# Vigilans/GomokuAI

Hardware: AMD Instinct MI355X
Metric: board-evals/s (higher is better)
Workload: dtype int32; 1 GPU; batched AC-automaton position eval (K1), 65536 random-opening boards per GPU, 15x15, inputs resident in HBM; boards_per_gpu=65536, parallelism=boards sharded by rank, no collective, launch=hipGraph replay of the K steps

## Files before the change

### gomokuai_amd/csrc/eval_kernel.hip

```cpp
#include <algorithm>
#include <cstdlib>
#include <vector>

#include "capi_common.h"
#include "host_staging.h"

namespace {

constexpr int kBoardsPerBlock = 16;
constexpr int kGroupBoards = 16;
constexpr int kThreads = 64 * kBoardsPerBlock;
constexpr int kCells = 225;
constexpr int kQueueCap = 448;
constexpr int kMaxBlocksPerCu = 1;
constexpr int kBurstEvery = 12;
static_assert(kBurstEvery >= 1 && kBurstEvery <= kGroupBoards, "every burst of a run needs a board of the run to go with");
[[maybe_unused]] constexpr int kTimelineSlots = 8;

constexpr int kScoreWords = 4 * kCells;
constexpr int kCntWords = 3 * kCells + 1;
constexpr int kZeroWords = kScoreWords + kCntWords;
constexpr int kLineWords = 96;
constexpr int kColBase = 20, kDiagBase = 36, kAntiBase = 65;
#ifndef GMK_K1_TOTALS_COPIES
#define GMK_K1_TOTALS_COPIES 8
#endif
constexpr int kTotalsCopies = GMK_K1_TOTALS_COPIES;
constexpr int kMiscWords = 48;
constexpr int kBoardWords = kZeroWords + kLineWords + kQueueCap + kMiscWords;
static_assert(kZeroWords % 4 == 0 && kBoardWords % 4 == 0, "16-byte alignment of the per-board blocks");
constexpr int kStaticTableWords = 128 + kLineWords + 512 + 1560 + 4;

constexpr int kLaneRecordVecs = 2;
constexpr int kScanSteps = 19;

__device__ __forceinline__ int dir_stride(int dir) { return (0x0E100F01u >> (8 * dir)) & 0xFFu; }

__device__ __forceinline__ uint64_t line_symbols(uint32_t line_word, int len) {
    return 2ull | (static_cast<uint64_t>(line_word) << 2) | (0xAull << (2 * len + 2));
}

__device__ __forceinline__ const __attribute__((address_space(3))) uint32_t* lds_word(uint32_t byte_address) {
    return reinterpret_cast<const __attribute__((address_space(3))) uint32_t*>(static_cast<uintptr_t>(byte_address));
}

__device__ __forceinline__ __attribute__((address_space(3))) uint32_t* lds_word_rw(uint32_t byte_address) {
    return reinterpret_cast<__attribute__((address_space(3))) uint32_t*>(static_cast<uintptr_t>(byte_address));
}

__device__ __forceinline__ uint32_t dfa_address(uint32_t table_word, uint32_t four) {
    uint32_t addr;
    asm("v_bfi_b32 %0, %1, %2, %3" : "=v"(addr) : "s"(0x3FF3u), "v"(table_word), "v"(four));
    return addr;
}

typedef unsigned short v2u16 __attribute__((ext_vector_type(2)));
__device__ __forceinline__ uint32_t pk_dec_u16(uint32_t word) {
    const v2u16 ones = {1, 1};
    return __builtin_bit_cast(uint32_t, static_cast<v2u16>(__builtin_bit_cast(v2u16, word) - ones));
}

__device__ __forceinline__ void store_saddr(uint32_t byte_offset, int32_t value, unsigned long long base) {
    asm volatile("global_store_dword %0, %1, %2" : : "v"(byte_offset), "v"(value), "s"(base) : "memory");
}

template <int kImm, bool kNt>
__device__ __forceinline__ void store_saddr_imm(uint32_t byte_offset, int32_t value, unsigned long long base) {
    static_assert(kImm >= 0 && kImm < 4096, "the immediate offset of a global store has 13 bits, signed");
    if (kNt) asm volatile("global_store_dword %0, %1, %2 offset:%3 nt" : : "v"(byte_offset), "v"(value), "s"(base), "n"(kImm) : "memory");
    else asm volatile("global_store_dword %0, %1, %2 offset:%3" : : "v"(byte_offset), "v"(value), "s"(base), "n"(kImm) : "memory");
}

__device__ __forceinline__ void wave_phase_fence() {
    __builtin_amdgcn_fence(__ATOMIC_RELEASE, "wavefront");
    __builtin_amdgcn_wave_barrier();
    __builtin_amdgcn_fence(__ATOMIC_ACQUIRE, "wavefront");
}

__device__ __forceinline__ void deposit_match(uint32_t w0, uint32_t w1, int cell_at, int dir, int back_step,
                                              uint32_t* s_scores, uint32_t* s_cnt, uint32_t* s_misc, uint32_t* totals ) {
    const int type = w0 & 15, fav = (w0 >> 4) & 1;
    if (type == 8) { atomicOr(&s_misc[1], fav ? 1u : 2u); return; }
    atomicAdd(&totals[type], fav ? 0x10000u : 1u);
    const int endcell = cell_at + static_cast<int>((w0 >> 27) & 1u) * back_step;
    const uint32_t score = dir >= 2 ? (w1 >> 16) : (w1 & 0xFFFFu);
    unsigned long long* pair = reinterpret_cast<unsigned long long*>(s_scores) + fav;
    const uint32_t lo_opp = fav ? score : 0u, hi_opp = fav ? 0u : score;
    const uint32_t tslot = 5u - static_cast<uint32_t>(type);
    const bool feeds = tslot < 3u;
    uint32_t* cnt = s_cnt + (feeds ? tslot : 0u) * kCells;
    const uint32_t one = 1u << (4 * (fav * 4 + dir));
    const int n_dep = (w0 >> 8) & 7;
#pragma unroll
    for (int d = 0; d < 4; ++d) {
        if (d >= n_dep) break;
        const uint32_t f = (w0 >> (11 + 4 * d)) & 15u;
        const int c = endcell + static_cast<int>(f & 7u) * back_step;
        const bool both = (f & 8u) != 0u;
        atomicAdd(&pair[2 * c], (static_cast<unsigned long long>(both ? score : hi_opp) << 32) | (both ? score : lo_opp));
        if (both && feeds) atomicAdd(&cnt[c], one);
    }
}

__device__ __forceinline__ int counter_match(uint32_t w0, int k, int want) {
    const int type = w0 & 15, len = (w0 >> 5) & 7;
    const int back = k - static_cast<int>((w0 >> 27) & 1u) - 6;
    if (!w0 || type != want || back < 0 || back >= len) return -1;
    const int n_dep = (w0 >> 8) & 7;
    bool on_q = false;
#pragma unroll
    for (int d = 0; d < 4; ++d) {
        const uint32_t f = (w0 >> (11 + 4 * d)) & 15u;
        on_q |= d < n_dep && f == (8u | static_cast<uint32_t>(back));
    }
    return on_q ? back : -1;
}

__device__ __forceinline__ void add_counter_cells(uint32_t w0, int back, int q, int stride, uint32_t* opp) {
    const int n_dep = (w0 >> 8) & 7, endcell = q + back * stride;
#pragma unroll
    for (int d = 0; d < 4; ++d) {
        const uint32_t f = (w0 >> (11 + 4 * d)) & 15u;
// ... 71 lines not shown
    }
    if ((lane & 33) == 0) {
        const int bg = lane >> 1;
        uint32_t* slot = s_occ + 8 * ((bg >> 1) & 1) + 2 * (bg >> 2) + (bg & 1);
#pragma unroll
        for (int m = 0; m < kDensTiles; ++m) {
            const int y0 = (32 * m) / 15, y1 = (32 * m + 31) / 15;
            uint32_t occ = 0;
#pragma unroll
            for (int y = y0; y <= y1; ++y) {
                const uint32_t both = own[y / 2] | other[y / 2];
                const uint32_t r = ((y & 1) ? both >> 16 : both) & 0x7FFFu;
                const int at = 15 * y - 32 * m;
                occ |= at >= 0 ? r << at : r >> -at;
            }
            slot[16 * m] = occ;
        }
    }
    if ((lane >> 5) == 0 && (kFull || (board < n_boards && plane_stride > 0))) {
        uint32_t c224 = 0, w224 = 0;
#pragma unroll
        for (int dy = -3; dy <= 0; ++dy) {
            const int y = 14 + dy;
            const uint32_t r = (y & 1) ? own[y >> 1] >> 16 : own[y >> 1] & 0xFFFFu;
#pragma unroll
            for (int dx = -3; dx <= 0; ++dx) {
                if (block_weight(dy, dx) == 0) continue;
                const uint32_t bit = (r >> (14 + dx)) & 1u;
                c224 += bit;
                w224 += bit * static_cast<uint32_t>(block_weight(dy, dx));
            }
        }
        const uint32_t neg = 0u - (((own[7] | other[7]) >> 14) & 1u);
        int32_t* out = out_density + static_cast<size_t>(board) * 4 * plane_stride + (1 - plane) * 2 * plane_stride;
        out[224] = static_cast<int32_t>(c224 ^ neg);
        out[plane_stride + 224] = static_cast<int32_t>(w224 ^ neg);
    }
    const int n_live = __builtin_amdgcn_readfirstlane(n_boards - first_board);
    int32_t* group_out = out_density + static_cast<size_t>(first_board) * 4 * plane_stride;
    const uint4* occ_words = reinterpret_cast<const uint4*>(s_occ);
    const unsigned long long group_bits = reinterpret_cast<unsigned long long>(group_out);
    unsigned long long board_base = static_cast<unsigned long long>(static_cast<uint32_t>(__builtin_amdgcn_readfirstlane(static_cast<int>(group_bits >> 32)))) << 32
                                    | static_cast<uint32_t>(__builtin_amdgcn_readfirstlane(static_cast<int>(group_bits)));
    asm volatile("" : "+s"(board_base));
#define GMK_PASS(K, M) density_tile_pass<kFull, K, M>(own, n_live, lane, s_wtab, occ_words, group_out, board_base, s_lut, plane_stride); __builtin_amdgcn_sched_barrier(0);
    GMK_PASS(0, 0) GMK_PASS(1, 0) GMK_PASS(0, 1) GMK_PASS(1, 1) GMK_PASS(0, 2) GMK_PASS(1, 2) GMK_PASS(0, 3) GMK_PASS(1, 3)
    GMK_PASS(0, 4) GMK_PASS(1, 4) GMK_PASS(0, 5) GMK_PASS(1, 5) GMK_PASS(0, 6) GMK_PASS(1, 6)
#undef GMK_PASS
}

__global__ __launch_bounds__(kThreads)
void eval_positions_kernel(const uint16_t* __restrict__ planes, int n_boards, int groups_each, int groups_extra,
                           int32_t* __restrict__ out_scores, int32_t* __restrict__ out_density,
                           uint32_t* __restrict__ out_totals, int32_t* __restrict__ out_status,
                           const uint4* __restrict__ g_stage, int stage_vecs, int trans_words, int record_words,
                           int phase_mask_arg, unsigned long long* __restrict__ prof, unsigned long long* __restrict__ timeline) {
#ifdef GMK_PROFILE
    unsigned long long* const tl_row = timeline ? timeline + (static_cast<size_t>(blockIdx.x) * kBoardsPerBlock + (threadIdx.x >> 6)) * kTimelineSlots : nullptr;
#define GMK_TL(slot, value) do { if (tl_row && (threadIdx.x & 63) == 0) tl_row[slot] = (value); } while (0)
    GMK_TL(0, __builtin_amdgcn_s_memtime());
    unsigned long long tl_last_board = 0, tl_burst_clocks = 0;
    int tl_bursts = 0;
    const int phase_mask = phase_mask_arg;
    unsigned long long t_acc[12] = {0, 0, 0, 0, 0, 0, 0, 0, 0, 0, 0, 0}, t_prev = __builtin_amdgcn_s_memtime();
#define GMK_STAMP(k) do { if (prof) { const unsigned long long t_now_ = __builtin_amdgcn_s_memtime(); t_acc[k] += t_now_ - t_prev; t_prev = t_now_; } } while (0)
#else
    constexpr int phase_mask = 0x7F;
    (void)phase_mask_arg; (void)prof; (void)timeline;
#define GMK_TL(slot, value) do { } while (0)
#ifdef GMK_K1_MARKERS
#define GMK_STAMP(k) asm volatile("; gmk_mark " #k)
#else
#define GMK_STAMP(k) do { } while (0)
#endif
#endif
    extern __shared__ __attribute__((aligned(16))) uint32_t lds[];
    const uint4* s_rec = reinterpret_cast<const uint4*>(lds + trans_words);
    uint32_t* s_jobs = lds + trans_words + record_words;

    const int tid = threadIdx.x;
    const uint4 stage_a = g_stage[min(tid, stage_vecs - 1)], stage_b = g_stage[min(tid + kThreads, stage_vecs - 1)];
    const uint4* lane_record = g_stage + stage_vecs + kLaneRecordVecs * (tid & 63);
    const uint4 lane_lines = lane_record[0], lane_consts = lane_record[1];
    uint32_t* s_pads = s_jobs + 128;
    uint2* s_lut = reinterpret_cast<uint2*>(s_jobs + 128 + kLineWords);
    uint32_t* s_wtab_words = s_jobs + 128 + kLineWords + 512;
    const v4i* s_wtab = reinterpret_cast<const v4i*>(s_wtab_words);
    uint32_t* s_handout = s_wtab_words + kWtabWords;

    const int wave = __builtin_amdgcn_readfirstlane(threadIdx.x >> 6), lane0 = threadIdx.x & 63;
    uint32_t* s_scores = lds + trans_words + record_words + kStaticTableWords + wave * kBoardWords;
    uint32_t* s_cnt = s_scores + kScoreWords;
    uint32_t* s_lines = s_scores + kZeroWords;
    uint32_t* s_queue = s_lines + kLineWords;
    uint32_t* s_misc = s_queue + kQueueCap;
#ifndef GMK_K1_TOTALS_HOT
    uint32_t* const my_totals = s_queue + kQueueCap - 8 * kTotalsCopies + (lane0 & (kTotalsCopies - 1)) * 8;
#else
    uint32_t* const my_totals = s_misc + 4;
#endif

    GMK_STAMP(0);

    const bool planes_out = out_density != nullptr && (phase_mask & 64) && !(phase_mask & 1024);
    int lane = lane0;
    const uint32_t job_a = lane_lines.x, job_b = lane_lines.y;
    const uint32_t line_init_lo = lane_lines.z, line_init_hi = lane_lines.w;
    const uint32_t cell_row4 = lane_consts.x, cell_col = lane_consts.y, norm_a = lane_consts.z, norm_b = lane_consts.w;
    uint32_t* s_rows = s_misc + 16;
    const uint16_t* row_ptr = planes + (lane & 15);
    uint32_t next_black = 0, next_white = 0, cur_black = 0, cur_white = 0;
    auto fetch_row = [&](int b) {
        const uint16_t* p = row_ptr + static_cast<size_t>(min(b, n_boards - 1)) * 32;
        next_black = p[0];
        next_white = p[16];
    };
    auto take_row = [&](int lane_m, int b) -> uint32_t { return lane_m < 16 && b < n_boards ? cur_black | (cur_white << 16) : 0u; };

    const int wg_block = static_cast<int>(blockIdx.x);
    const int wg_g0 = groups_each * wg_block + min(wg_block, groups_extra);
    const int wg_groups = groups_each + (wg_block < groups_extra ? 1 : 0);
    const int wg_first = wg_g0 * kGroupBoards, wg_boards = min(wg_groups * kGroupBoards, n_boards - wg_first);
    auto hand_out = [&]() -> int {
        uint32_t v = 0;
        if (lane0 == 0) v = atomicAdd(s_handout, 1u);
        return __builtin_amdgcn_readfirstlane(static_cast<int>(v));
    };
    int idx = wave, boards_done = 0;
    if (idx < wg_boards) fetch_row(wg_first + idx);
    {
        uint4* s_stage = reinterpret_cast<uint4*>(lds);
        if (tid < stage_vecs) s_stage[tid] = stage_a;
        if (tid + kThreads < stage_vecs) s_stage[tid + kThreads] = stage_b;
        for (int i = tid + 2 * kThreads; i < stage_vecs; i += kThreads) s_stage[i] = g_stage[i];
    }
    asm volatile("" : "+v"(next_black), "+v"(next_white));
    GMK_TL(1, __builtin_amdgcn_s_memtime());
#pragma unroll 1
    for (;;) {
#ifdef GMK_K1_MARKERS
        GMK_STAMP(10);
#endif
        const bool live = idx < wg_boards;
        const int board = wg_first + idx;
        cur_black = next_black; cur_white = next_white;
        int idx_next = idx;
        if (live) { idx_next = boards_done == 0 ? kBoardsPerBlock + wave : hand_out(); fetch_row(wg_first + min(idx_next, wg_boards - 1)); }
        GMK_STAMP(11);

        if (live) {
            {
                uint4* z = reinterpret_cast<uint4*>(s_cnt) + lane;
    #pragma unroll
                for (int i = 0; i < kCntWords / 4; i += 64)
                    if (i + 64 <= kCntWords / 4 || lane < kCntWords / 4 - i) z[i] = make_uint4(0u, 0u, 0u, 0u);
            }
            int lane_m = lane;
            asm volatile("" : "+v"(lane_m));
            s_lines[lane] = line_init_lo;
            if (lane_m < kLineWords - 64) s_lines[64 + lane] = line_init_hi;
            if (lane_m < kMiscWords) s_misc[lane] = 0;
#ifndef GMK_K1_TOTALS_HOT
            if (lane < 8 * kTotalsCopies) s_queue[kQueueCap - 8 * kTotalsCopies + lane] = 0;
#endif
            const uint32_t my_row = take_row(lane_m, board);
            wave_phase_fence();
            {
                uint32_t cnt = static_cast<uint32_t>(__popc(my_row & 0x7FFFu)) | (static_cast<uint32_t>(__popc(my_row >> 16)) << 16);
                cnt += static_cast<uint32_t>(__builtin_amdgcn_update_dpp(0, static_cast<int>(cnt), 0x118, 0xF, 0xF, false));
                cnt += static_cast<uint32_t>(__builtin_amdgcn_update_dpp(0, static_cast<int>(cnt), 0x114, 0xF, 0xF, false));
                cnt += static_cast<uint32_t>(__builtin_amdgcn_update_dpp(0, static_cast<int>(cnt), 0x112, 0xF, 0xF, false));
                cnt += static_cast<uint32_t>(__builtin_amdgcn_update_dpp(0, static_cast<int>(cnt), 0x111, 0xF, 0xF, false));
                if (lane_m == 15) s_misc[0] = cnt;
            }
            {
                const uint32_t r = my_row;
                const v2u16 rr = __builtin_bit_cast(v2u16, r);
                const uint32_t l1 = __builtin_bit_cast(uint32_t, static_cast<v2u16>(rr << 1)), l2 = __builtin_bit_cast(uint32_t, static_cast<v2u16>(rr << 2)), l3 = __builtin_bit_cast(uint32_t, static_cast<v2u16>(rr << 3));
                const uint32_t r1 = __builtin_bit_cast(uint32_t, static_cast<v2u16>(rr >> 1)), r2 = __builtin_bit_cast(uint32_t, static_cast<v2u16>(rr >> 2)), r3 = __builtin_bit_cast(uint32_t, static_cast<v2u16>(rr >> 3));
                const int far = static_cast<int>(r | l3 | r3), near = static_cast<int>(r | l1 | l2 | r1 | r2);
                uint32_t g = l1 | l2 | l3 | r1 | r2 | r3;
                g |= static_cast<uint32_t>(__builtin_amdgcn_update_dpp(0, near, 0x111, 0xF, 0xF, true)) | static_cast<uint32_t>(__builtin_amdgcn_update_dpp(0, near, 0x101, 0xF, 0xF, true));
                g |= static_cast<uint32_t>(__builtin_amdgcn_update_dpp(0, near, 0x112, 0xF, 0xF, true)) | static_cast<uint32_t>(__builtin_amdgcn_update_dpp(0, near, 0x102, 0xF, 0xF, true));
                g |= static_cast<uint32_t>(__builtin_amdgcn_update_dpp(0, far, 0x113, 0xF, 0xF, true)) | static_cast<uint32_t>(__builtin_amdgcn_update_dpp(0, far, 0x103, 0xF, 0xF, true));
                const uint32_t empty = ~(r | (r >> 16)) & 0x7FFFu;
                if (lane < 15) s_rows[3 + lane] = r;
                const int gate = static_cast<int>(g & (empty | (empty << 16)));
    #pragma unroll
                for (int pass = 0; pass < 4; ++pass) {
                    const uint32_t gw = static_cast<uint32_t>(__builtin_amdgcn_ds_bpermute(static_cast<int>((cell_row4 >> (8 * pass)) & 0xFFu), gate)) >> ((cell_col >> (8 * pass)) & 0xFFu);
                    if (pass < 3 || lane < kCells - 192)
                        reinterpret_cast<uint4*>(s_scores)[64 * pass + lane] = make_uint4(static_cast<uint32_t>(__builtin_amdgcn_sbfe(static_cast<int>(gw), 16, 1)) & 160u, 0u, 0u,
                                                                                          static_cast<uint32_t>(__builtin_amdgcn_sbfe(static_cast<int>(gw), 0, 1)) & 160u);
                }
            }
            {
                const int y = lane >> 2, part = lane & 3;
                const uint32_t row = __shfl(my_row, min(y, 14));
                uint32_t row_sym = 0;
                uint32_t y2 = 2u * static_cast<uint32_t>(y), y4 = 4u * static_cast<uint32_t>(y);
                asm volatile("" : "+v"(y2), "+v"(y4));
                for (uint32_t m = lane < 60 ? (row | (row >> 16)) & (0xFu << (4 * part)) & 0x7FFFu : 0u; m; m &= m - 1u) {
                    const int x = __ffs(m) - 1;
                    const uint32_t code = ((row >> x) & 1u) | 2u;
                    const uint32_t at_x = code << (2 * x), at_y = code << y2;
                    row_sym |= at_x;
                    char* const col = reinterpret_cast<char*>(s_lines + x);
                    atomicXor(reinterpret_cast<uint32_t*>(col) + kColBase, at_y);
                    atomicXor(reinterpret_cast<uint32_t*>(col - y4) + (kDiagBase + 14), at_x);
                    atomicXor(reinterpret_cast<uint32_t*>(col + y4) + kAntiBase, at_y);
                }
                if (row_sym) atomicXor(&s_lines[y], row_sym);
            }
            wave_phase_fence();
            GMK_STAMP(1);
        }
#ifdef GMK_PROFILE
        if (boards_done == 0) GMK_TL(2, __builtin_amdgcn_s_memtime());
#endif
        if (boards_done == 0) __syncthreads();
#ifdef GMK_PROFILE
        if (boards_done == 0) GMK_TL(3, __builtin_amdgcn_s_memtime());
        if (live) { tl_bursts = 0; tl_burst_clocks = 0; }
#endif
        if (live) {
            int n_queued = 0;
            if (phase_mask & 2) {
                const int len_a = static_cast<int>(job_a & 31u) - 3, len_b = static_cast<int>(job_b & 31u) - 3;
                uint64_t syms = line_symbols(s_lines[(job_a >> 20) & 127u] >> norm_a, len_a);
                syms |= line_symbols(s_lines[(job_b >> 20) & 127u] >> norm_b, len_b) << (2 * len_a + 6);
                syms |= 0xAAAAAAAAAAAAAAAAull << (2 * (len_a + len_b) + 12);
                const uint32_t cur = static_cast<uint32_t>(syms) << 2;
                const uint32_t rest = static_cast<uint32_t>(syms >> 28);
                uint32_t tw = 0;
                const uint32_t q_base = static_cast<uint32_t>(s_queue - lds) * 4u;
                const uint32_t q_full = q_base + 4u * (kQueueCap - 64);
                uint32_t q_at = q_base;
                auto push = [&](uint32_t word, int step) {
                    const bool emits = word > 0x1FFFFu;
                    const unsigned long long emitters = __ballot(emits);
                    if (emitters) {
                        if (emits) {
                            const uint32_t ahead = __builtin_amdgcn_mbcnt_hi(static_cast<uint32_t>(emitters >> 32), __builtin_amdgcn_mbcnt_lo(static_cast<uint32_t>(emitters), 0u));
                            *lds_word_rw(q_at + 4u * ahead) = (word & ~0x1FFFFu) | (static_cast<uint32_t>(lane) | static_cast<uint32_t>(step) << 6);
                        }
                        q_at = min(q_at + 4u * static_cast<uint32_t>(__popcll(emitters)), q_full);
                    }
                };
#pragma unroll
                for (int step = 0; step < kScanSteps; ++step) {
                    const uint32_t four = step < 15 ? __builtin_amdgcn_ubfe(cur, 2 * step, 4) : __builtin_amdgcn_ubfe(rest, 2 * (step - 15), 4);
                    const uint32_t addr = dfa_address(tw, four);
                    const uint32_t before = tw;
                    tw = *lds_word(addr);
                    if (step > 0) push(before, step - 1);
                }
                push(tw, kScanSteps - 1);
                n_queued = static_cast<int>((q_at - q_base) >> 2);
                if (q_at >= q_full) s_misc[2] = 1;
            }
            wave_phase_fence();
            GMK_STAMP(2);

            if (phase_mask & 4) {
                uint32_t qe_next = s_queue[min(lane, kQueueCap - 1)];
                for (int m = lane; m < n_queued; m += 64) {
                    const uint32_t qe = qe_next;
                    qe_next = s_queue[min(m + 64, kQueueCap - 1)];
                    const int src_lane = qe & 63, src_step = (qe >> 6) & 31;
                    const uint4 rec_now = s_rec[qe >> 17];
                    const uint32_t ja_now = s_jobs[src_lane * 2], jb_now = s_jobs[src_lane * 2 + 1];
                    const int seg_a = ja_now & 31u;
                    const bool second = src_step >= seg_a;
                    const uint32_t job = second ? jb_now : ja_now;
                    const int pos = src_step - 1 - (second ? seg_a : 0);
                    const int dir = (job >> 5) & 3, stride = (job >> 7) & 31;
                    const int cell_at = static_cast<int>((job >> 12) & 255u) + pos * stride;
                    deposit_match(rec_now.x, rec_now.y, cell_at, dir, -stride, s_scores, s_cnt, s_misc, my_totals);
                    if (rec_now.z) deposit_match(rec_now.z, rec_now.w, cell_at, dir, -stride, s_scores, s_cnt, s_misc, my_totals);
                }
            }
            wave_phase_fence();
#ifndef GMK_K1_TOTALS_HOT
            if (lane < 8) {
                const uint32_t* t = s_queue + kQueueCap - 8 * kTotalsCopies + lane;
                uint32_t sum = 0;
#pragma unroll
                for (int c = 0; c < kTotalsCopies; ++c) sum += t[8 * c];
                s_misc[4 + lane] = sum;
            }
#endif
            GMK_STAMP(3);

            int n_cand = 0;
            if (phase_mask & 8) {
                uint32_t any_cnt[4];
    #pragma unroll
                for (int pass = 0; pass < 4; ++pass) {
                    const int qc = min(64 * pass + lane, kCells - 1);
                    any_cnt[pass] = s_cnt[qc] | s_cnt[kCells + qc] | s_cnt[2 * kCells + qc];
                }
    #pragma unroll
                for (int pass = 0; pass < 4; ++pass) {
                    const int q = 64 * pass + lane;
                    const uint32_t any = any_cnt[pass];
                    const uint32_t hot = any & (pk_dec_u16(any) | 0xEEEEEEEEu);
                    const unsigned long long pushers = __ballot(hot != 0u) & (pass < 3 ? ~0ull : (1ull << (kCells - 192)) - 1ull);
                    if (pushers) {
                        if (hot != 0u && (pass < 3 || lane < kCells - 192)) {
                            const int slot = n_cand + static_cast<int>(__builtin_amdgcn_mbcnt_hi(static_cast<uint32_t>(pushers >> 32),
                                                                       __builtin_amdgcn_mbcnt_lo(static_cast<uint32_t>(pushers), 0u)));
                            if (slot < kQueueCap / 2) s_queue[slot] = static_cast<uint32_t>(q) | ((hot & 0xFFFFu) ? 0x100u : 0u) | ((hot >> 16) ? 0x200u : 0u);
                        }
                        n_cand += __popcll(pushers);
                    }
                }
            }
            wave_phase_fence();
            GMK_STAMP(4);

            if (n_cand > kQueueCap / 2) { s_misc[2] = 1; n_cand = kQueueCap / 2; }
            if (phase_mask & 2048) n_cand = 0;
            constexpr int kRescanFlush = kQueueCap / 2 - 2 * 64;
            static_assert(kRescanFlush > 0 && kRescanFlush + 2 * 64 <= kQueueCap / 2, "a round of phase 3b fits behind the flush level");
            int n_comp_q = 0;
            if (phase_mask & 8)
            for (int v0 = 0; v0 < 2 * n_cand; v0 += 64) {
                const int v = v0 + lane;
                const int flag_shift = 8 + (v & 1);
                const uint32_t ce = s_queue[v >> 1];
                const int q = ce & 255, c = v & 1;
                bool queue = false;
                uint32_t ent1 = 0, ent2 = 0;
                if (v < 2 * n_cand && ((ce >> flag_shift) & 1u)) {
                    const uint32_t f3 = (s_cnt[q] >> (16 * c)) & 0xFFFFu, fd = (s_cnt[kCells + q] >> (16 * c)) & 0xFFFFu, f2 = (s_cnt[2 * kCells + q] >> (16 * c)) & 0xFFFFu;
                    uint32_t dens = 0;
                    const int qy = (q * 0x8889) >> 19, qx = q - 15 * qy;
                    {
                        const int half = c ? 0 : 16;
    #pragma unroll
                        for (int dy = -3; dy <= 3; ++dy) {
                            const uint32_t pattern = dy == 0 ? 0x77u : (dy == 3 || dy == -3) ? 0x49u : 0x3Eu;
                            const uint32_t mask = ((pattern << qx) >> 3) & 0x7FFFu;
                            dens += __popc((s_rows[3 + qy + dy] >> half) & mask);
                        }
                    }
                    if (dens >= 2u) {
                        const uint32_t up3 = (f3 >> 1) | (f3 >> 2) | (f3 >> 3), upd = (fd >> 1) | (fd >> 2) | (fd >> 3), up2 = (f2 >> 1) | (f2 >> 2) | (f2 >> 3);
                        const uint32_t sel3 = (f3 | up3) & 0x1111u;
                        const uint32_t seld = (fd | upd) & 0x1111u & ~sel3;
                        const uint32_t sel2 = (f2 | up2) & 0x1111u & ~(sel3 | seld);
                        const uint32_t strong = sel3 | seld, any_dir = strong | sel2;
                        const uint32_t twice_strong = (sel3 & up3) | (seld & upd), twice = twice_strong | (sel2 & up2);
                        const int n_comp = __popc(any_dir) + __popc(twice), threes = __popc(strong) + __popc(twice_strong);
                        if (n_comp < 2) {
                            s_misc[2] = 1;
                        } else {
                            const int ctype = min(threes, 2);
// ... 84 lines not shown
#endif
            int lane_p = lane0, first_p = (wg_g0 + burst) * kGroupBoards;
            asm volatile("" : "+v"(lane_p), "+s"(first_p));
            const int plane_stride = (phase_mask & 512) ? 0 : (phase_mask & 256) ? 256 : kCells;
            if (first_p + kGroupBoards <= n_boards && plane_stride > 0) density_planes_out<true>(planes, n_boards, first_p, lane_p, s_wtab, s_queue, out_density, s_lut, plane_stride);
            else density_planes_out<false>(planes, n_boards, first_p, lane_p, s_wtab, s_queue, out_density, s_lut, plane_stride);
            GMK_STAMP(8);
#ifdef GMK_PROFILE
            ++tl_bursts; tl_burst_clocks += __builtin_amdgcn_s_memtime() - tl_burst_from;
#endif
        }
#ifdef GMK_K1_MARKERS
        GMK_STAMP(12);
#endif
        if (live && (phase_mask & 32)) {
            int lane_b = lane;
            asm volatile("" : "+v"(lane_b));
            const uint32_t lane_off = 4u * static_cast<uint32_t>(lane_b);
            if (out_scores) {
                const unsigned long long dst = reinterpret_cast<unsigned long long>(out_scores + static_cast<size_t>(board) * kScoreWords);
                const int4* src = reinterpret_cast<const int4*>(s_scores);
                const int4 v0 = src[lane_b], v1 = src[lane_b + 64], v2 = src[lane_b + 128], v3 = src[min(lane_b + 192, kCells - 1)];
#ifdef GMK_K1_PLAIN_SCORES
                constexpr bool kNt = false;
#else
                constexpr bool kNt = true;
#endif
#define GMK_STORE(words, v) store_saddr_imm<4 * (words), kNt>(lane_off, v, dst)
                const bool tail = lane_b + 192 < kCells;
                GMK_STORE(0, v0.x); GMK_STORE(64, v1.x); GMK_STORE(128, v2.x); if (tail) GMK_STORE(192, v3.x);
                GMK_STORE(kCells, v0.y); GMK_STORE(kCells + 64, v1.y); GMK_STORE(kCells + 128, v2.y); if (tail) GMK_STORE(kCells + 192, v3.y);
                GMK_STORE(2 * kCells, v0.z); GMK_STORE(2 * kCells + 64, v1.z); GMK_STORE(2 * kCells + 128, v2.z); if (tail) GMK_STORE(2 * kCells + 192, v3.z);
                GMK_STORE(3 * kCells, v0.w); GMK_STORE(3 * kCells + 64, v1.w); GMK_STORE(3 * kCells + 128, v2.w); if (tail) GMK_STORE(3 * kCells + 192, v3.w);
#undef GMK_STORE
            }
            if (out_totals) {
                const unsigned long long dst = reinterpret_cast<unsigned long long>(out_totals + static_cast<size_t>(board) * 11);
                if (lane_b < 11) store_saddr_imm<0, false>(lane_off, static_cast<int32_t>(s_misc[4 + lane_b]), dst);
            }
            if (out_status) {
                const uint32_t stones = static_cast<uint32_t>(__builtin_amdgcn_readfirstlane(static_cast<int>(s_misc[0])));
                const uint32_t wbits = static_cast<uint32_t>(__builtin_amdgcn_readfirstlane(static_cast<int>(s_misc[1])));
                const uint32_t flagged = static_cast<uint32_t>(__builtin_amdgcn_readfirstlane(static_cast<int>(s_misc[2])));
                const int stones_b = stones & 0xFFFFu, stones_w = stones >> 16;
                const int winner = (wbits & 1u) ? 1 : (wbits & 2u) ? -1 : 0;
                const bool over = winner != 0 || stones_b + stones_w == kCells;
                const int to_move = over ? 0 : (stones_b == stones_w ? 1 : -1);
                const int word = (over ? 1 : 0) | ((flagged || phase_mask != 0x7F) ? 2 : 0) | ((winner & 0xFF) << 8) | ((to_move & 0xFF) << 16);
                const unsigned long long dst = reinterpret_cast<unsigned long long>(out_status + board);
                if (lane_b == 0) store_saddr_imm<0, false>(lane_off, word, dst);
            }
        }
        wave_phase_fence();
        GMK_STAMP(9);
#ifdef GMK_PROFILE
        tl_last_board = __builtin_amdgcn_s_memtime();
#endif
        idx = idx_next; ++boards_done;
    }
#ifdef GMK_PROFILE
    GMK_TL(4, tl_last_board);
    GMK_TL(6, static_cast<unsigned long long>(tl_bursts) | static_cast<unsigned long long>(boards_done) << 16);
    GMK_TL(7, tl_burst_clocks);
    GMK_TL(5, __builtin_amdgcn_s_memtime());
    if (prof && lane0 == 0) {
        for (int k = 0; k < 12; ++k) atomicAdd(&prof[k], t_acc[k]);
        atomicAdd(&prof[15], 1ull);
    }
#endif
#undef GMK_STAMP
#undef GMK_TL
}

struct LineJob { int len, x0, y0, dir; };

int lane_tables(uint32_t* jobs_out, uint32_t* pads_out, uint32_t* records_out) {
    std::vector<LineJob> lines;
    for (int i = 0; i < 15; ++i) lines.push_back({15, 0, i, 0});
    for (int i = 0; i < 15; ++i) lines.push_back({15, i, 0, 1});
    for (int d = -10; d <= 10; ++d) lines.push_back({15 - std::abs(d), d > 0 ? d : 0, d > 0 ? 0 : -d, 2});
    for (int k = 4; k <= 24; ++k) { const int x0 = std::min(k, 14); lines.push_back({std::min(k, 28 - k) + 1, x0, k - x0, 3}); }
    std::stable_sort(lines.begin(), lines.end(), [](const LineJob& a, const LineJob& b) { return a.len > b.len; });
    uint32_t jobs[128];
    for (uint32_t& j : jobs) j = 3u | (15u << 20);
    auto pack = [](const LineJob& l) {
        const int line = l.dir == 0 ? l.y0 : l.dir == 1 ? kColBase + l.x0 : l.dir == 2 ? kDiagBase + l.x0 - l.y0 + 14 : kAntiBase + l.x0 + l.y0;
        const int stride = l.dir == 0 ? 1 : l.dir == 1 ? 15 : l.dir == 2 ? 16 : 14;
        return static_cast<uint32_t>((l.len + 3) | (l.dir << 5) | (stride << 7) | ((l.y0 * 15 + l.x0) << 12) | (line << 20));
    };
    int steps = 0;
    for (int lane = 0; lane < 64; ++lane) {
        jobs[lane * 2] = pack(lines[lane]);
        int total = lines[lane].len + 3;
        const int extra = 64 + (63 - lane);
        if (extra < static_cast<int>(lines.size())) { jobs[lane * 2 + 1] = pack(lines[extra]); total += lines[extra].len + 3; }
        steps = std::max(steps, total);
    }
    uint32_t init[kLineWords] = {};
    for (int i = 0; i < 15; ++i) init[i] = init[kColBase + i] = 0x3FFFFFFFu;
    for (int d = 0; d <= 28; ++d) init[kDiagBase + d] = init[kAntiBase + d] = ((1u << (2 * (15 - std::abs(d - 14)))) - 1u) << (2 * std::max(0, d - 14));
    uint32_t consts[64][4];
    for (int lane = 0; lane < 64; ++lane) {
        uint32_t row4 = 0, col = 0;
        for (int pass = 0; pass < 4; ++pass) {
            const int c = std::min(64 * pass + lane, kCells - 1);
            row4 |= static_cast<uint32_t>(4 * (c / 15)) << (8 * pass);
            col |= static_cast<uint32_t>(c % 15) << (8 * pass);
        }
        consts[lane][0] = row4;
        consts[lane][1] = col;
        for (int k = 0; k < 2; ++k) {
            const uint32_t job = jobs[lane * 2 + k], dir = (job >> 5) & 3u, first = (job >> 12) & 255u;
            consts[lane][2 + k] = dir == 2u ? 2u * (first % 15u) : dir == 3u ? 2u * (first / 15u) : 0u;
        }
    }
    for (int i = 0; i < 128; ++i) jobs_out[i] = jobs[i];
    for (int i = 0; i < kLineWords; ++i) pads_out[i] = ~init[i] & 0xAAAAAAAAu;
    for (int lane = 0; lane < 64; ++lane) {
        uint32_t* r = records_out + 8 * lane;
        r[0] = jobs[lane * 2]; r[1] = jobs[lane * 2 + 1];
        r[2] = init[lane]; r[3] = init[std::min(64 + lane, kLineWords - 1)];
        for (int k = 0; k < 4; ++k) r[4 + k] = consts[lane][k];
    }
    if (steps != kScanSteps) { gmk::set_error("lane jobs: %d scan steps, the kernel is built for %d", steps, kScanSteps); return GMK_ERR_STATE; }
    return GMK_OK;
}

int density_weights(int8_t* t ) {
    for (int kind = 0; kind < 2; ++kind)
        for (int dy = -3; dy <= 3; ++dy)
            for (int xo = 0; xo < 15; ++xo)
                for (int j = 0; j < 15; ++j) {
                    if (std::abs(j - xo) > 3) continue;
                    const int w = block_weight(dy, j - xo);
                    t[((static_cast<size_t>(kind) * kWtabDy + dy + 6) * 15 + xo) * 16 + j] = static_cast<int8_t>(kind == 0 ? (w != 0) : w);
                }
    for (int cell = 0; cell < 224; ++cell)
        for (int kt = dens_kt_lo(cell / 32); kt <= dens_kt_hi(cell / 32); ++kt)
            for (int h = 0; h < 2; ++h) {
                const int dy = 2 * kt + h - cell / 15;
                if (dy < -6 || dy > 6) { gmk::set_error("density weight table: dy %d of cell %d out of range", dy, cell); return GMK_ERR_STATE; }
            }
    for (int cell = 0; cell < 224; ++cell)
        for (int dy = -3; dy <= 3; ++dy) {
            const int y = cell / 15 + dy, m = cell / 32;
            if (y < 0 || y > 14) continue;
            if (y / 2 < dens_kt_lo(m) || y / 2 > dens_kt_hi(m)) { gmk::set_error("density weight table: row %d of cell %d is not covered", y, cell); return GMK_ERR_STATE; }
        }
    return GMK_OK;
}

int build_stage_image(const gmk::DeviceState& st, uint4** d_out, int* stage_vecs) {
    const size_t trans_words = static_cast<size_t>(st.n_states) * 4, record_words = static_cast<size_t>(st.n_records) * 4;
    std::vector<uint32_t> rest(kStaticTableWords + 64 * 4 * kLaneRecordVecs, 0u);
    uint32_t* jobs = rest.data(), *pads = jobs + 128, *lut = pads + kLineWords, *wtab = lut + 512, *handout = wtab + kWtabWords, *records = handout + 4;
    int rc = lane_tables(jobs, pads, records);
    if (rc != GMK_OK) return rc;
    for (uint32_t b = 0; b < 256; ++b) { lut[2 * b] = ((b & 15u) * 0x204081u) & 0x01010101u; lut[2 * b + 1] = ((b >> 4) * 0x204081u) & 0x01010101u; }
    rc = density_weights(reinterpret_cast<int8_t*>(wtab));
    if (rc != GMK_OK) return rc;
    handout[0] = 2u * kBoardsPerBlock;
    const size_t staged_words = trans_words + record_words + kStaticTableWords;
    if (staged_words % 4 != 0) { gmk::set_error("K1 tables: %zu staged words are not whole 16-byte pieces", staged_words); return GMK_ERR_STATE; }
    uint32_t* d = nullptr;
    GMK_HIP_CHECK(hipMalloc(&d, (trans_words + record_words + rest.size()) * sizeof(uint32_t)));
    GMK_HIP_CHECK(hipMemcpy(d, st.d_trans, trans_words * sizeof(uint32_t), hipMemcpyDeviceToDevice));
    GMK_HIP_CHECK(hipMemcpy(d + trans_words, st.d_records, record_words * sizeof(uint32_t), hipMemcpyDeviceToDevice));
    GMK_HIP_CHECK(hipMemcpy(d + trans_words + record_words, rest.data(), rest.size() * sizeof(uint32_t), hipMemcpyHostToDevice));
    *d_out = reinterpret_cast<uint4*>(d);
    *stage_vecs = static_cast<int>(staged_words / 4);
    return GMK_OK;
}

struct Launch { int grid, n_groups, groups_each, groups_extra; size_t lds; };

Launch plan_launch(int n, const gmk::DeviceState& st) {
    Launch l;
    l.n_groups = (n + kGroupBoards - 1) / kGroupBoards;
    l.grid = std::max(1, std::min(l.n_groups, st.cu_count * kMaxBlocksPerCu));
    l.groups_each = l.n_groups / l.grid;
    l.groups_extra = l.n_groups % l.grid;
    l.lds = static_cast<size_t>(kBoardsPerBlock * kBoardWords + st.n_states * 4 + st.n_records * 4 + kStaticTableWords) * 4;
    return l;
}

bool g_jobs_uploaded = false;
uint4* g_stage = nullptr;
int g_stage_vecs = 0;
}

extern "C" int gmk_eval_batch(const uint16_t* d_planes, int n, int32_t* d_scores, int32_t* d_density,
                              uint32_t* d_totals, int32_t* d_status, void* stream) {
    gmk::DeviceState& st = gmk::device_state();
    GMK_NEED_INIT();
    if (n < 0 || (n > 0 && !d_planes)) { gmk::set_error("gmk_eval_batch: bad arguments"); return GMK_ERR_ARG; }
    if (n == 0) return GMK_OK;
    if (!g_jobs_uploaded) {
        const int rc = build_stage_image(st, &g_stage, &g_stage_vecs);
        if (rc != GMK_OK) return rc;
        GMK_HIP_CHECK(hipFuncSetAttribute(reinterpret_cast<const void*>(eval_positions_kernel), hipFuncAttributeMaxDynamicSharedMemorySize, 160 * 1024));
        g_jobs_uploaded = true;
    }
    const Launch l = plan_launch(n, st);
    if (l.lds > 160u * 1024u) { gmk::set_error("gmk_eval_batch: tables do not fit in LDS (%zu bytes)", l.lds); return GMK_ERR_CAPACITY; }
    static const int phase_mask = gmk::profile_env("GMK_EVAL_PHASE_MASK") ? std::atoi(gmk::profile_env("GMK_EVAL_PHASE_MASK")) : 0x7F;
    unsigned long long* d_prof = nullptr;
    static const bool stamps = gmk::profile_env("GMK_EVAL_PROFILE") != nullptr;
    if (stamps) {
        GMK_HIP_CHECK(hipMalloc(&d_prof, 16 * sizeof(unsigned long long)));
        GMK_HIP_CHECK(hipMemset(d_prof, 0, 16 * sizeof(unsigned long long)));
    }
    static const char* const timeline_path = gmk::profile_env("GMK_EVAL_TIMELINE");
    unsigned long long* d_timeline = nullptr;
    const size_t timeline_words = static_cast<size_t>(l.grid) * kBoardsPerBlock * kTimelineSlots;
    hipEvent_t tl_from = nullptr, tl_to = nullptr;
    if (timeline_path) {
        GMK_HIP_CHECK(hipMalloc(&d_timeline, timeline_words * sizeof(unsigned long long)));
        GMK_HIP_CHECK(hipMemset(d_timeline, 0, timeline_words * sizeof(unsigned long long)));
        GMK_HIP_CHECK(hipEventCreate(&tl_from));
        GMK_HIP_CHECK(hipEventCreate(&tl_to));
        GMK_HIP_CHECK(hipDeviceSynchronize());
        GMK_HIP_CHECK(hipEventRecord(tl_from, static_cast<hipStream_t>(stream)));
    }
    hipLaunchKernelGGL(eval_positions_kernel, dim3(l.grid), dim3(kThreads), l.lds, static_cast<hipStream_t>(stream),
                       d_planes, n, l.groups_each, l.groups_extra, d_scores, d_density, d_totals, d_status,
                       g_stage, g_stage_vecs, st.n_states * 4, st.n_records * 4, phase_mask, d_prof, d_timeline);
    GMK_HIP_CHECK(hipGetLastError());
    if (timeline_path) {
        GMK_HIP_CHECK(hipEventRecord(tl_to, static_cast<hipStream_t>(stream)));
        GMK_HIP_CHECK(hipEventSynchronize(tl_to));
        float wall_ms = 0.f;
        GMK_HIP_CHECK(hipEventElapsedTime(&wall_ms, tl_from, tl_to));
        std::vector<unsigned long long> h(4 + timeline_words);
        h[0] = static_cast<unsigned long long>(l.grid); h[1] = kBoardsPerBlock; h[2] = kTimelineSlots; h[3] = static_cast<unsigned long long>(wall_ms * 1e6);
        GMK_HIP_CHECK(hipMemcpy(h.data() + 4, d_timeline, timeline_words * sizeof(unsigned long long), hipMemcpyDeviceToHost));
        (void)hipFree(d_timeline); (void)hipEventDestroy(tl_from); (void)hipEventDestroy(tl_to);
        if (std::FILE* f = std::fopen(timeline_path, "wb")) { std::fwrite(h.data(), sizeof(unsigned long long), h.size(), f); std::fclose(f); }
    }
    if (stamps) {
        unsigned long long h[16];
        GMK_HIP_CHECK(hipDeviceSynchronize());
        GMK_HIP_CHECK(hipMemcpy(h, d_prof, sizeof h, hipMemcpyDeviceToHost));
        (void)hipFree(d_prof);
        const char* names[12] = {"staging", "phase0", "scan", "deposits", "phase3", "phase3b", "rescans", "wait-planes", "phaseD", "phase5", "-", "loop-head"};
// ... 40 lines not shown
```

Measured before the change: 589.3 million board-evals/s.

## Shorten AC scan with precomputed start state and interleave board setup into lookups

Each line segment now uses two pad symbols instead of three. The scan starts from a host-verified state reached after the leading '?' pad, and the host checks that "??" from any state resyncs to that state. This cuts the per-lane DFA scan from 19 to 17 dependent LDS lookups. The per-board setup work (counter clearing, stone count, gate computation, score seeding) is split into ten pieces that run between the serial DFA lookups with sched barriers, to hide the lookup latency. The cost is correctness that depends on automaton properties checked at build time, plus a tighter instruction schedule that may raise register pressure.

```diff
diff --git a/gomokuai_amd/csrc/eval_kernel.hip b/gomokuai_amd/csrc/eval_kernel.hip
--- a/gomokuai_amd/csrc/eval_kernel.hip
+++ b/gomokuai_amd/csrc/eval_kernel.hip
@@ -32,12 +32,13 @@
 constexpr int kStaticTableWords = 128 + kLineWords + 512 + 1560 + 4;
 
 constexpr int kLaneRecordVecs = 2;
-constexpr int kScanSteps = 19;
+constexpr int kSegPads = 2;
+constexpr int kScanSteps = 17;
 
 __device__ __forceinline__ int dir_stride(int dir) { return (0x0E100F01u >> (8 * dir)) & 0xFFu; }
 
 __device__ __forceinline__ uint64_t line_symbols(uint32_t line_word, int len) {
-    return 2ull | (static_cast<uint64_t>(line_word) << 2) | (0xAull << (2 * len + 2));
+    return static_cast<uint64_t>(line_word) | (0xAull << (2 * len));
 }
 
 __device__ __forceinline__ const __attribute__((address_space(3))) uint32_t* lds_word(uint32_t byte_address) {
@@ -275,6 +276,7 @@
     const uint4 stage_a = g_stage[min(tid, stage_vecs - 1)], stage_b = g_stage[min(tid + kThreads, stage_vecs - 1)];
     const uint4* lane_record = g_stage + stage_vecs + kLaneRecordVecs * (tid & 63);
     const uint4 lane_lines = lane_record[0], lane_consts = lane_record[1];
+    const uint32_t scan_start = reinterpret_cast<const uint32_t*>(g_stage)[trans_words + record_words + kStaticTableWords - 3];
     uint32_t* s_pads = s_jobs + 128;
     uint2* s_lut = reinterpret_cast<uint2*>(s_jobs + 128 + kLineWords);
     uint32_t* s_wtab_words = s_jobs + 128 + kLineWords + 512;
@@ -341,33 +343,27 @@
         if (live) { idx_next = boards_done == 0 ? kBoardsPerBlock + wave : hand_out(); fetch_row(wg_first + min(idx_next, wg_boards - 1)); }
         GMK_STAMP(11);
 
-        if (live) {
-            {
-                uint4* z = reinterpret_cast<uint4*>(s_cnt) + lane;
-    #pragma unroll
-                for (int i = 0; i < kCntWords / 4; i += 64)
-                    if (i + 64 <= kCntWords / 4 || lane < kCntWords / 4 - i) z[i] = make_uint4(0u, 0u, 0u, 0u);
-            }
-            int lane_m = lane;
-            asm volatile("" : "+v"(lane_m));
-            s_lines[lane] = line_init_lo;
-            if (lane_m < kLineWords - 64) s_lines[64 + lane] = line_init_hi;
-            if (lane_m < kMiscWords) s_misc[lane] = 0;
+        uint32_t late_row = 0;
+        int late_lane = lane, late_gate = 0;
+        auto late_piece = [&](int piece) {
+            if (piece == 0) {
 #ifndef GMK_K1_TOTALS_HOT
-            if (lane < 8 * kTotalsCopies) s_queue[kQueueCap - 8 * kTotalsCopies + lane] = 0;
-#endif
-            const uint32_t my_row = take_row(lane_m, board);
-            wave_phase_fence();
-            {
-                uint32_t cnt = static_cast<uint32_t>(__popc(my_row & 0x7FFFu)) | (static_cast<uint32_t>(__popc(my_row >> 16)) << 16);
+                if (lane < 8 * kTotalsCopies) s_queue[kQueueCap - 8 * kTotalsCopies + lane] = 0;
+#endif
+            } else if (piece <= 3) {
+                constexpr int kVecs = kCntWords / 4;
+                static_assert(kVecs > 128 && kVecs <= 192, "three pieces of 64 lanes clear the counters");
+                const int i = 64 * (piece - 1);
+                if (i + 64 <= kVecs || late_lane < kVecs - i) (reinterpret_cast<uint4*>(s_cnt) + lane)[i] = make_uint4(0u, 0u, 0u, 0u);
+            } else if (piece == 4) {
+                uint32_t cnt = static_cast<uint32_t>(__popc(late_row & 0x7FFFu)) | (static_cast<uint32_t>(__popc(late_row >> 16)) << 16);
                 cnt += static_cast<uint32_t>(__builtin_amdgcn_update_dpp(0, static_cast<int>(cnt), 0x118, 0xF, 0xF, false));
                 cnt += static_cast<uint32_t>(__builtin_amdgcn_update_dpp(0, static_cast<int>(cnt), 0x114, 0xF, 0xF, false));
                 cnt += static_cast<uint32_t>(__builtin_amdgcn_update_dpp(0, static_cast<int>(cnt), 0x112, 0xF, 0xF, false));
                 cnt += static_cast<uint32_t>(__builtin_amdgcn_update_dpp(0, static_cast<int>(cnt), 0x111, 0xF, 0xF, false));
-                if (lane_m == 15) s_misc[0] = cnt;
-            }
-            {
-                const uint32_t r = my_row;
+                if (late_lane == 15) s_misc[0] = cnt;
+            } else if (piece == 5) {
+                const uint32_t r = late_row;
                 const v2u16 rr = __builtin_bit_cast(v2u16, r);
                 const uint32_t l1 = __builtin_bit_cast(uint32_t, static_cast<v2u16>(rr << 1)), l2 = __builtin_bit_cast(uint32_t, static_cast<v2u16>(rr << 2)), l3 = __builtin_bit_cast(uint32_t, static_cast<v2u16>(rr << 3));
                 const uint32_t r1 = __builtin_bit_cast(uint32_t, static_cast<v2u16>(rr >> 1)), r2 = __builtin_bit_cast(uint32_t, static_cast<v2u16>(rr >> 2)), r3 = __builtin_bit_cast(uint32_t, static_cast<v2u16>(rr >> 3));
@@ -378,15 +374,26 @@
                 g |= static_cast<uint32_t>(__builtin_amdgcn_update_dpp(0, far, 0x113, 0xF, 0xF, true)) | static_cast<uint32_t>(__builtin_amdgcn_update_dpp(0, far, 0x103, 0xF, 0xF, true));
                 const uint32_t empty = ~(r | (r >> 16)) & 0x7FFFu;
                 if (lane < 15) s_rows[3 + lane] = r;
-                const int gate = static_cast<int>(g & (empty | (empty << 16)));
-    #pragma unroll
-                for (int pass = 0; pass < 4; ++pass) {
-                    const uint32_t gw = static_cast<uint32_t>(__builtin_amdgcn_ds_bpermute(static_cast<int>((cell_row4 >> (8 * pass)) & 0xFFu), gate)) >> ((cell_col >> (8 * pass)) & 0xFFu);
-                    if (pass < 3 || lane < kCells - 192)
-                        reinterpret_cast<uint4*>(s_scores)[64 * pass + lane] = make_uint4(static_cast<uint32_t>(__builtin_amdgcn_sbfe(static_cast<int>(gw), 16, 1)) & 160u, 0u, 0u,
-                                                                                          static_cast<uint32_t>(__builtin_amdgcn_sbfe(static_cast<int>(gw), 0, 1)) & 160u);
-                }
-            }
+                late_gate = static_cast<int>(g & (empty | (empty << 16)));
+            } else if (piece <= 9) {
+                const int pass = piece - 6;
+                const uint32_t gw = static_cast<uint32_t>(__builtin_amdgcn_ds_bpermute(static_cast<int>((cell_row4 >> (8 * pass)) & 0xFFu), late_gate)) >> ((cell_col >> (8 * pass)) & 0xFFu);
+                if (pass < 3 || lane < kCells - 192)
+                    reinterpret_cast<uint4*>(s_scores)[64 * pass + lane] = make_uint4(static_cast<uint32_t>(__builtin_amdgcn_sbfe(static_cast<int>(gw), 16, 1)) & 160u, 0u, 0u,
+                                                                                      static_cast<uint32_t>(__builtin_amdgcn_sbfe(static_cast<int>(gw), 0, 1)) & 160u);
+            }
+        };
+        constexpr int kLatePieces = 10;
+        static_assert(kLatePieces <= kScanSteps, "a piece per lookup");
+        if (live) {
+            int lane_m = lane;
+            asm volatile("" : "+v"(lane_m));
+            s_lines[lane] = line_init_lo;
+            if (lane_m < kLineWords - 64) s_lines[64 + lane] = line_init_hi;
+            if (lane_m < kMiscWords) s_misc[lane] = 0;
+            const uint32_t my_row = take_row(lane_m, board);
+            late_row = my_row; late_lane = lane_m;
+            wave_phase_fence();
             {
                 const int y = lane >> 2, part = lane & 3;
                 const uint32_t row = __shfl(my_row, min(y, 14));
@@ -419,13 +426,13 @@
         if (live) {
             int n_queued = 0;
             if (phase_mask & 2) {
-                const int len_a = static_cast<int>(job_a & 31u) - 3, len_b = static_cast<int>(job_b & 31u) - 3;
+                const int len_a = static_cast<int>(job_a & 31u) - kSegPads, len_b = static_cast<int>(job_b & 31u) - kSegPads;
                 uint64_t syms = line_symbols(s_lines[(job_a >> 20) & 127u] >> norm_a, len_a);
-                syms |= line_symbols(s_lines[(job_b >> 20) & 127u] >> norm_b, len_b) << (2 * len_a + 6);
-                syms |= 0xAAAAAAAAAAAAAAAAull << (2 * (len_a + len_b) + 12);
+                syms |= line_symbols(s_lines[(job_b >> 20) & 127u] >> norm_b, len_b) << (2 * (len_a + kSegPads));
+                syms |= 0xAAAAAAAAAAAAAAAAull << (2 * (len_a + len_b + 2 * kSegPads));
                 const uint32_t cur = static_cast<uint32_t>(syms) << 2;
                 const uint32_t rest = static_cast<uint32_t>(syms >> 28);
-                uint32_t tw = 0;
+                uint32_t tw = scan_start;
                 const uint32_t q_base = static_cast<uint32_t>(s_queue - lds) * 4u;
                 const uint32_t q_full = q_base + 4u * (kQueueCap - 64);
                 uint32_t q_at = q_base;
@@ -446,12 +453,20 @@
                     const uint32_t addr = dfa_address(tw, four);
                     const uint32_t before = tw;
                     tw = *lds_word(addr);
+                    if (step < kLatePieces) __builtin_amdgcn_sched_barrier(0);
                     if (step > 0) push(before, step - 1);
+                    if (step < kLatePieces) { late_piece(step); __builtin_amdgcn_sched_barrier(0); }
                 }
                 push(tw, kScanSteps - 1);
                 n_queued = static_cast<int>((q_at - q_base) >> 2);
                 if (q_at >= q_full) s_misc[2] = 1;
             }
+#ifdef GMK_PROFILE
+            else {
+#pragma unroll
+                for (int piece = 0; piece < kLatePieces; ++piece) late_piece(piece);
+            }
+#endif
             wave_phase_fence();
             GMK_STAMP(2);
 
@@ -466,7 +481,7 @@
                     const int seg_a = ja_now & 31u;
                     const bool second = src_step >= seg_a;
                     const uint32_t job = second ? jb_now : ja_now;
-                    const int pos = src_step - 1 - (second ? seg_a : 0);
+                    const int pos = src_step - (second ? seg_a : 0);
                     const int dir = (job >> 5) & 3, stride = (job >> 7) & 31;
                     const int cell_at = static_cast<int>((job >> 12) & 255u) + pos * stride;
                     deposit_match(rec_now.x, rec_now.y, cell_at, dir, -stride, s_scores, s_cnt, s_misc, my_totals);
@@ -717,18 +732,18 @@
     for (int k = 4; k <= 24; ++k) { const int x0 = std::min(k, 14); lines.push_back({std::min(k, 28 - k) + 1, x0, k - x0, 3}); }
     std::stable_sort(lines.begin(), lines.end(), [](const LineJob& a, const LineJob& b) { return a.len > b.len; });
     uint32_t jobs[128];
-    for (uint32_t& j : jobs) j = 3u | (15u << 20);
+    for (uint32_t& j : jobs) j = static_cast<uint32_t>(kSegPads) | (15u << 20);
     auto pack = [](const LineJob& l) {
         const int line = l.dir == 0 ? l.y0 : l.dir == 1 ? kColBase + l.x0 : l.dir == 2 ? kDiagBase + l.x0 - l.y0 + 14 : kAntiBase + l.x0 + l.y0;
         const int stride = l.dir == 0 ? 1 : l.dir == 1 ? 15 : l.dir == 2 ? 16 : 14;
-        return static_cast<uint32_t>((l.len + 3) | (l.dir << 5) | (stride << 7) | ((l.y0 * 15 + l.x0) << 12) | (line << 20));
+        return static_cast<uint32_t>((l.len + kSegPads) | (l.dir << 5) | (stride << 7) | ((l.y0 * 15 + l.x0) << 12) | (line << 20));
     };
     int steps = 0;
     for (int lane = 0; lane < 64; ++lane) {
         jobs[lane * 2] = pack(lines[lane]);
-        int total = lines[lane].len + 3;
+        int total = lines[lane].len + kSegPads;
         const int extra = 64 + (63 - lane);
-        if (extra < static_cast<int>(lines.size())) { jobs[lane * 2 + 1] = pack(lines[extra]); total += lines[extra].len + 3; }
+        if (extra < static_cast<int>(lines.size())) { jobs[lane * 2 + 1] = pack(lines[extra]); total += lines[extra].len + kSegPads; }
         steps = std::max(steps, total);
     }
     uint32_t init[kLineWords] = {};
@@ -785,6 +800,23 @@
     return GMK_OK;
 }
 
+int scan_start_row(const gmk::DeviceTables& t, uint32_t* row_out) {
+    constexpr uint32_t kPad = 2;
+    const std::vector<uint32_t>& tr = t.dev_trans;
+    const uint32_t n = static_cast<uint32_t>(t.n_states);
+    if (n == 0 || tr.size() != static_cast<size_t>(n) * 4) { gmk::set_error("K1 scan: no automaton"); return GMK_ERR_STATE; }
+    const uint32_t first = tr[kPad], start = gmk::dev_trans_row(first);
+    if (gmk::dev_trans_record(first) != 0 || start % 16 != 0 || start / 16 >= n) { gmk::set_error("K1 scan: the root emits on '?' or leaves the table"); return GMK_ERR_STATE; }
+    const uint32_t loop = tr[start / 4 + kPad];
+    if (gmk::dev_trans_record(loop) != 0 || gmk::dev_trans_row(loop) != start) { gmk::set_error("K1 scan: state %u does not loop on '?' without emitting", start / 16); return GMK_ERR_STATE; }
+    for (uint32_t s = 0; s < n; ++s) {
+        const uint32_t mid = gmk::dev_trans_row(tr[s * 4 + kPad]);
+        if (mid % 16 != 0 || mid / 16 >= n || gmk::dev_trans_row(tr[mid / 4 + kPad]) != start) { gmk::set_error("K1 scan: \"??\" from state %u does not lead to state %u", s, start / 16); return GMK_ERR_STATE; }
+    }
+    *row_out = start;
+    return GMK_OK;
+}
+
 int build_stage_image(const gmk::DeviceState& st, uint4** d_out, int* stage_vecs) {
     const size_t trans_words = static_cast<size_t>(st.n_states) * 4, record_words = static_cast<size_t>(st.n_records) * 4;
     std::vector<uint32_t> rest(kStaticTableWords + 64 * 4 * kLaneRecordVecs, 0u);
@@ -795,6 +827,8 @@
     rc = density_weights(reinterpret_cast<int8_t*>(wtab));
     if (rc != GMK_OK) return rc;
     handout[0] = 2u * kBoardsPerBlock;
+    rc = scan_start_row(gmk::production_automaton().device(), &handout[1]);
+    if (rc != GMK_OK) return rc;
     const size_t staged_words = trans_words + record_words + kStaticTableWords;
     if (staged_words % 4 != 0) { gmk::set_error("K1 tables: %zu staged words are not whole 16-byte pieces", staged_words); return GMK_ERR_STATE; }
     uint32_t* d = nullptr;
```

Result: faster. 600.6 million board-evals/s (median of 6 runs) (+1.9%).
